# xbpeng/DeepTerrainRL

Hardware: AMD Instinct MI355X
Metric: env-steps/sec (batched rollout) dog/slopes_mixed (higher is better)
Workload: dtype f64

## Files before the change

### deepterrainrl_amd/csrc/dtrl_kernel_fast.h

```cpp
#pragma once
#include "dtrl_kernel.h"
#include "dtrl_topo.h"
#include <type_traits>

#if defined(__HIP_DEVICE_COMPILE__)

#if !DTRL_WAVE_SYNC
#error "dtrl_kernel_fast.h: the register-resident path is ONE wavefront per env by construction (v_readlane broadcasts, ballots, and LDS read-then-write sequences such as warm_match_fast() that rely on a wave's LDS operations completing in issue order). -DDTRL_WAVE_SYNC=0 builds the lane-phase reference path only (ADVICE r5)"
#endif

namespace dtrl {

__device__ __forceinline__ int lane_id() { return static_cast<int>(threadIdx.x); }
__device__ __forceinline__ int opaque_lane()
{
	int lane = static_cast<int>(threadIdx.x);
	asm volatile("" : "+v"(lane));
	return lane;
}
template <class T>
__device__ __forceinline__ void pin_loaded(T& v) { asm volatile("" : "+v"(v)); }
#if defined(DTRL_REAL_F32)
#define DTRL_VFMA "v_fma_f32"
#define DTRL_VMOV "v_mov_b32"
#else
#define DTRL_VFMA "v_fma_f64"
#define DTRL_VMOV "v_mov_b64"
#endif
__device__ __forceinline__ real bcast(real v, int src)
{
#if defined(DTRL_REAL_F32)
	return __int_as_float(__builtin_amdgcn_readlane(__float_as_int(v), src));
#else
	int lo = __builtin_amdgcn_readlane(__double2loint(v), src);
	int hi = __builtin_amdgcn_readlane(__double2hiint(v), src);
	return __hiloint2double(hi, lo);
#endif
}

template <int D>
__device__ __forceinline__ void mass_row(WSFast& ws, real (&h)[D])
{
	constexpr int Lk = D - 2;
	constexpr int kTab = Lk * (Lk + 5) / 2;
	constexpr int kFill = (kTab + 1) & ~1;
	static_assert(kFill <= static_cast<int>(sizeof(ws.Apk) / sizeof(real)), "mass table does not fit the packed-matrix storage");
	const int d = static_cast<int>(threadIdx.x);
	const int l = d >= 2 ? d - 2 : 0;
	const bool hinge = d >= 2 && d < D;
	real* T = ws.Apk;
	{
		struct alignas(2 * sizeof(real)) real2 { real x, y; };
		real2* T2 = reinterpret_cast<real2*>(T);
		const real2 z2 = {0.0, 0.0};
#pragma unroll
		for (int e = 0; e < (kFill / 2 + kGroup - 1) / kGroup; ++e) if (d + e * kGroup < kFill / 2) T2[d + e * kGroup] = z2;
	}
	env_sync();
	if (hinge) {
		const int base = l * (l + 5) / 2;
		const real m = ws.sm[l], mx = ws.smx[l], my = ws.smy[l];
		T[base] = -(my - m * ws.py[l]);
		T[base + 1] = (mx - m * ws.px[l]);
	}
	const int n_pairs = ws.M.n_pairs;
#pragma unroll 2
	for (int e = lane_id(); e < n_pairs; e += kGroup) {
		const int pl = ws.M.pair_l[e], pk = ws.M.pair_k[e];
		const int a = ws.M.path[pl][pk];
		const real m = ws.sm[pl], mx = ws.smx[pl], my = ws.smy[pl], I = ws.sI[pl];
		const real plx = ws.px[pl], ply = ws.py[pl];
		const real pax = ws.px[a], pay = ws.py[a];
		T[pl * (pl + 5) / 2 + 2 + a] = I - ((plx + pax) * mx + (ply + pay) * my) + m * (plx * pax + ply * pay);
	}
	env_sync();
	const real M0 = ws.sm[0];
	const real* Tl = T + (d < D ? d : 0);
	h[0] = (d == 0) ? M0 : 0.0;
	h[1] = (d == 1) ? M0 : 0.0;
#pragma unroll
	for (int c = 2; c < D; ++c) h[c] = Tl[(c - 2) * (c + 3) / 2];
	env_sync();
}

template <int B, int E, class F>
__device__ __forceinline__ void static_for(F&& f)
{
	if constexpr (B < E) { f(std::integral_constant<int, B>{}); static_for<B + 1, E>(f); }
}
template <int B, int E, class F>
__device__ __forceinline__ void static_for_down(F&& f)
{
	if constexpr (B < E) { f(std::integral_constant<int, E - 1>{}); static_for_down<B, E - 1>(f); }
}
template <int J>
__device__ __forceinline__ void fnma_lanes_ge(real& acc, real a, real b)
{
	unsigned long long sv, m;
	asm("s_lshl_b64 %2, -1, %5\n\ts_and_saveexec_b64 %1, %2\n\t" DTRL_VFMA " %0, -%3, %4, %0\n\ts_mov_b64 exec, %1"
	    : "+v"(acc), "=&s"(sv), "=&s"(m) : "v"(a), "s"(b), "n"(J) : "scc");
}
template <int I>
__device__ __forceinline__ void fnma_lanes_lt(real& acc, real a, real b)
{
	unsigned long long sv, m;
	asm("s_bfm_b64 %2, %5, 0\n\ts_and_saveexec_b64 %1, %2\n\t" DTRL_VFMA " %0, -%3, %4, %0\n\ts_mov_b64 exec, %1"
	    : "+v"(acc), "=&s"(sv), "=&s"(m) : "v"(a), "s"(b), "n"(I) : "scc");
}
template <int K>
__device__ __forceinline__ void mov_lane_eq(real& dst, real src)
{
	unsigned long long sv, m;
	asm("s_lshl_b64 %2, 1, %4\n\ts_and_saveexec_b64 %1, %2\n\t" DTRL_VMOV " %0, %3\n\ts_mov_b64 exec, %1"
	    : "+v"(dst), "=&s"(sv), "=&s"(m) : "v"(src), "n"(K) : "scc");
}
template <int I>
__device__ __forceinline__ void mov_lanes_lt(real& dst, real src)
{
	unsigned long long sv, m;
	asm("s_bfm_b64 %2, %4, 0\n\ts_and_saveexec_b64 %1, %2\n\t" DTRL_VMOV " %0, %3\n\ts_mov_b64 exec, %1"
	    : "+v"(dst), "=&s"(sv), "=&s"(m) : "v"(src), "n"(I) : "scc");
}
template <int B, int E>
__device__ __forceinline__ void mov_lanes_in(real& dst, real src)
{
	static_assert(0 <= B && B < E && E <= 64 && E - B < 64, "lane window (s_bfm_b64 takes the width modulo 64)");
	unsigned long long sv, m;
	asm("s_bfm_b64 %2, %4, %5\n\ts_and_saveexec_b64 %1, %2\n\t" DTRL_VMOV " %0, %3\n\ts_mov_b64 exec, %1"
	    : "+v"(dst), "=&s"(sv), "=&s"(m) : "v"(src), "n"(E - B), "n"(B) : "scc");
}
__device__ __forceinline__ void lds_store_ordered(real& dst, real v)
{
	dst = v;
	asm volatile("" : : : "memory");
}

template <class Topo>
__device__ __forceinline__ real factorize_regs(WSFast& ws, real (&h)[Topo::L + 2])
{
	constexpr int D = Topo::L + 2;
	const int lane = static_cast<int>(threadIdx.x);
	real dinv = 0;
	static_for_down<1, D>([&](auto kc) {
		constexpr int k = decltype(kc)::value;
		const real dk = bcast(h[k], k);
		const real ak = h[k];
		const real rk = fast_recip(dk);
		mov_lane_eq<k>(dinv, rk);
		const real lik = ak * rk;
		static_for_down<0, k>([&](auto jc) {
			constexpr int j = decltype(jc)::value;
			if constexpr (dof_coupled<Topo>(j, k)) h[j] = fmadd(-lik, bcast(ak, j), h[j]);
		});
		mov_lanes_lt<k>(h[k], lik);
	});
	{ const real r0 = fast_recip(h[0]); if (lane == 0) dinv = r0; }
	static_assert((D - 1) * (D - 2) / 2 + kGroup - 1 < static_cast<int>(sizeof(ws.Apk) / sizeof(real)), "the unpredicated store of U's last column leaves the packed-matrix storage");
	real* S = ws.Apk;
	static_for<1, D>([&](auto kc) {
		constexpr int k = decltype(kc)::value;
		lds_store_ordered(S[k * (k - 1) / 2 + lane], h[k]);
	});
	env_sync();
	const int base = lane < D ? lane * (lane - 1) / 2 : 0;
	static_for<0, D - 1>([&](auto kc) {
		constexpr int k = decltype(kc)::value;
		const real t = S[base + k];
		mov_lanes_in<k + 1, D>(h[k], t);
	});
	env_sync();
	return dinv;
}
template <int D>
__device__ __forceinline__ real usolve_regs(const real (&h)[D], real z)
{
	static_for_down<1, D>([&](auto kc) {
		constexpr int k = decltype(kc)::value;
		const real zk = bcast(z, k);
		fnma_lanes_lt<k>(z, h[k], zk);
	});
	return z;
}
template <class Topo>
constexpr int first_update_col(int i)
{
	for (int k = Topo::L + 1; k > i; --k) if (dof_coupled<Topo>(i, k)) return k;
	return 0;
}
template <class Topo, int kAhead = 1>
__device__ __forceinline__ void usolve_rows(WSFast& ws, int R)
{
	constexpr int D = Topo::L + 2;
	const int lane = static_cast<int>(threadIdx.x);
	if (lane > R) return;
	real* z = ws.Z[lane];
	const real* U = ws.Apk;
	real acc[D], u[D * (D - 1) / 2];
	auto fetch = [&](auto kc) {
		constexpr int k = decltype(kc)::value;
		static_for<0, k>([&](auto ic) {
			constexpr int i = decltype(ic)::value;
			if constexpr (dof_coupled<Topo>(i, k)) u[k * (k - 1) / 2 + i] = U[k * (k - 1) / 2 + i];
			if constexpr (first_update_col<Topo>(i) == k) acc[i] = z[i];
		});
		if constexpr (first_update_col<Topo>(k) == 0) acc[k] = z[k];
	};
	static_for_down<D - kAhead, D>(fetch);
	static_for_down<1, D>([&](auto kc) {
		constexpr int k = decltype(kc)::value;
		__builtin_amdgcn_sched_barrier(0);
		if constexpr (k - kAhead >= 1) fetch(std::integral_constant<int, k - kAhead>{});
		const real zk = acc[k];
		if constexpr (first_update_col<Topo>(k) != 0) z[k] = zk;
		static_for_down<0, k>([&](auto ic) {
			constexpr int i = decltype(ic)::value;
			if constexpr (dof_coupled<Topo>(i, k)) acc[i] = fmadd(-u[k * (k - 1) / 2 + i], zk, acc[i]);
		});
	});
	z[0] = acc[0];
}
template <int D>
__device__ __forceinline__ real utsolve_regs(const real (&h)[D], real u)
{
	static_for<0, D - 1>([&](auto kc) {
		constexpr int k = decltype(kc)::value;
		const real uk = bcast(u, k);
		fnma_lanes_ge<k + 1>(u, h[k], uk);
	});
	return u;
}

static_assert((kMaxPts + kGroup - 1) / kGroup == 3, "written for up to 3 sample points per lane");
constexpr int pts_per_lane(int L) { return (L * kPtsPerLink + kGroup - 1) / kGroup; }
struct ContactPts { PtVal p0, p1, p2; unsigned long long m0, m1, m2;  unsigned long long f0, f1, f2;  };
template <int NP>
__device__ __forceinline__ unsigned link_field(unsigned long long m0, unsigned long long m1, unsigned long long m2, int link)
{
	const int b = link * kPtsPerLink, word = b >> 6, off = b & 63;
	unsigned long long lo = m0, hi = NP > 1 ? m1 : 0ull;
	if constexpr (NP > 1) if (word == 1) { lo = m1; hi = NP > 2 ? m2 : 0ull; }
	if constexpr (NP > 2) if (word == 2) { lo = m2; hi = 0ull; }
	unsigned long long bits = lo >> off;
	if (off + kPtsPerLink > 64) bits |= hi << (64 - off);
	return static_cast<unsigned>(bits & ((1ull << kPtsPerLink) - 1ull));
}
constexpr real kNoPoint = -1.0e30;
template <int NP>
__device__ __noinline__ unsigned link_cap_drop_mask(WSFast& ws, real d0, real d1, real d2)
{
	const int lane = opaque_lane();
	const int npts = ws.M.L * kPtsPerLink;
	real* S = ws.Apk;
	if (lane < npts) S[lane] = d0;
	if constexpr (NP > 1) if (lane + kGroup < npts) S[lane + kGroup] = d1;
	if constexpr (NP > 2) if (lane + 2 * kGroup < npts) S[lane + 2 * kGroup] = d2;
	env_sync();
	auto over = [&](real d, int pt) -> unsigned {
		if (!(d > kNoPoint)) return 0u;
		const int base = (pt / kPtsPerLink) * kPtsPerLink;
		int rank = 0;
		for (int k = 0; k < kPtsPerLink; ++k) { const int o = base + k; const real od = S[o]; rank += (o != pt && (od > d || (od == d && o < pt))) ? 1 : 0; }
		return rank >= kMaxPtsPerLink ? 1u : 0u;
	};
	unsigned m = over(d0, lane);
	if constexpr (NP > 1) m |= over(d1, lane + kGroup) << 1;
	if constexpr (NP > 2) m |= over(d2, lane + 2 * kGroup) << 2;
	env_sync();
	return m;
}
template <int L, bool kFlags>
__device__ __forceinline__ ContactPts eval_points(WSFast& ws, const DevModel& gm, const GroundRec& g)
{
	constexpr int NP = pts_per_lane(L), npts = L * kPtsPerLink;
	const int lane = opaque_lane();
	const GroundHdr gh = ground_header(g);
	const real q0 = ws.st.q[0], q1 = ws.st.q[1];
	const real tol = kFlags ? gm.contact_tol : real(0);
	bool have[NP]; int col[NP]; real lx[NP], ly[NP], margin[NP], brk[NP], cs[NP], sn[NP], px[NP], py[NP];
	static_for<0, NP>([&](auto ec) {
		constexpr int e = decltype(ec)::value;
		const int pt = lane + e * kGroup;
		have[e] = (e + 1) * kGroup <= npts || pt < npts;
		const int ptc = ((e + 1) * kGroup <= npts || pt < npts) ? pt : npts - 1;
		const int j = ptc / kPtsPerLink;
		col[e] = ws.M.col[j];
		cs[e] = ws.cs[j]; sn[e] = ws.sn[j]; px[e] = ws.px[j]; py[e] = ws.py[j];
		const real* lp = &gm.pt_ground[0][0][0] + 2 * ptc;
		lx[e] = lp[0]; ly[e] = lp[1];
		margin[e] = gm.link_margin[j]; brk[e] = gm.link_brk[j];
	});
	static_for<0, NP>([&](auto ec) {
		constexpr int e = decltype(ec)::value;
		pin_loaded(col[e]); pin_loaded(lx[e]); pin_loaded(ly[e]); pin_loaded(margin[e]); pin_loaded(brk[e]);
	});
	real x[NP], y[NP]; GroundCell cell[NP];
	static_for<0, NP>([&](auto ec) {
		constexpr int e = decltype(ec)::value;
		x[e] = px[e] + cs[e] * lx[e] - sn[e] * ly[e];
		y[e] = py[e] + sn[e] * lx[e] + cs[e] * ly[e];
		cell[e] = ground_cell(gh, q0 + x[e]);
	});
	real ha[NP], hb[NP];
	static_for<0, NP>([&](auto ec) {
		constexpr int e = decltype(ec)::value;
		ha[e] = g.data[cell[e].seg][cell[e].i];
		hb[e] = g.data[cell[e].seg][cell[e].j];
	});
	PtVal r[3];
	static_for<0, 3>([&](auto ec) {
		constexpr int e = decltype(ec)::value;
		r[e].x = 0; r[e].y = 0; r[e].depth = 0; r[e].nx = 0; r[e].ny = 0; r[e].active = 0; r[e].near = 0;
		if constexpr (e < NP) {
			real slope;
			const real h = ground_height(cell[e], ha[e], hb[e], &slope);
			const real gap = h - (q1 + y[e]);
			const bool in_reach = kFlags || (gap + (margin[e] + brk[e]) * (1.0 + fabs(slope)) > 0);
			const real inv = fast_rsqrt(1.0 + slope * slope);
			const real depth = fmadd(gap, inv, margin[e]);
			const bool live = have[e] & (col[e] != 0);
			if (kFlags) r[e].near = (live & (depth >= -tol)) ? 1 : 0;
			r[e].active = (live & in_reach & (depth > -brk[e])) ? 1 : 0;
			r[e].nx = -slope * inv; r[e].ny = inv;
			r[e].depth = depth;
			r[e].x = x[e]; r[e].y = y[e];
		}
	});
	ContactPts c;
	c.p0 = r[0]; c.p1 = r[1]; c.p2 = r[2];
	c.f0 = 0; c.f1 = 0; c.f2 = 0;
	if (kFlags) { c.f0 = __ballot(c.p0.near); if constexpr (NP > 1) c.f1 = __ballot(c.p1.near); if constexpr (NP > 2) c.f2 = __ballot(c.p2.near); }
	c.m0 = __ballot(c.p0.active); c.m1 = 0; c.m2 = 0;
	if constexpr (NP > 1) c.m1 = __ballot(c.p1.active);
	if constexpr (NP > 2) c.m2 = __ballot(c.p2.active);
	if ((c.m0 | c.m1 | c.m2) != 0ull) {
		const int many = (lane < L) && __popc(link_field<NP>(c.m0, c.m1, c.m2, lane)) > kMaxPtsPerLink;
		if (__builtin_expect(__ballot(many) != 0ull, 0)) {
			const unsigned drop = link_cap_drop_mask<NP>(ws, c.p0.active ? c.p0.depth : kNoPoint, (NP > 1 && c.p1.active) ? c.p1.depth : kNoPoint, (NP > 2 && c.p2.active) ? c.p2.depth : kNoPoint);
			if (drop & 1u) c.p0.active = 0;
			if (drop & 2u) c.p1.active = 0;
			if (drop & 4u) c.p2.active = 0;
			c.m0 = __ballot(c.p0.active);
			if constexpr (NP > 1) c.m1 = __ballot(c.p1.active);
			if constexpr (NP > 2) c.m2 = __ballot(c.p2.active);
		}
	}
	return c;
}
template <int NP>
__device__ __noinline__ unsigned row_cap_drop_mask(WSFast& ws, real d0, real d1, real d2, int cap)
{
	const int lane = opaque_lane();
	const int npts = ws.M.L * kPtsPerLink;
	real* S = ws.Apk;
	if (lane < npts) S[lane] = d0;
	if constexpr (NP > 1) if (lane + kGroup < npts) S[lane + kGroup] = d1;
	if constexpr (NP > 2) if (lane + 2 * kGroup < npts) S[lane + 2 * kGroup] = d2;
	env_sync();
	auto over = [&](real d, int pt) -> unsigned {
		if (!(d > kNoPoint)) return 0u;
		int rank = 0;
		for (int o = 0; o < npts; ++o) { const real od = S[o]; rank += (o != pt && (od > d || (od == d && o < pt))) ? 1 : 0; }
		return rank >= cap ? 1u : 0u;
	};
	unsigned m = over(d0, lane);
	if constexpr (NP > 1) m |= over(d1, lane + kGroup) << 1;
	if constexpr (NP > 2) m |= over(d2, lane + 2 * kGroup) << 2;
	env_sync();
	return m;
}
__device__ __forceinline__ unsigned long long pairs_in_reach(const WSFast& ws)
{
	const int lane = static_cast<int>(threadIdx.x);
	return __ballot(lane < ws.M.n_cpairs && pair_in_reach(ws, lane));
}
constexpr int kPairCands = 2 * kPtsPerLink, kPairSlots = kGroup / kPairCands;
__device__ __noinline__ int append_pair_rows_fast(WSFast& ws, const DevModel& gm, int R, unsigned long long reach)
{
	const int lane = opaque_lane();
	const unsigned long long below = (lane == 0) ? 0ull : (~0ull >> (64 - lane));
	const int slot = lane / kPairCands, cand = lane - slot * kPairCands;
	while (reach != 0ull && R + 2 <= kMaxRows) {
		int mypr = -1;
#pragma unroll
		for (int sidx = 0; sidx < kPairSlots; ++sidx) {
			if (reach != 0ull) { const int pr = __ffsll(static_cast<long long>(reach)) - 1; reach &= reach - 1ull; if (slot == sidx) mypr = pr; }
		}
		int P = 0, Q = 0, k = 0;
		PairHit hit; hit.active = 0; hit.depth = 0; hit.x = 0; hit.y = 0; hit.nx = 0; hit.ny = 0;
		if (mypr >= 0) { pair_candidate(ws.M.cp_a[mypr], ws.M.cp_b[mypr], cand, &P, &Q, &k); hit = pair_point_eval(ws, gm, P, Q, k); }
		const unsigned long long am = __ballot(hit.active);
		if (am == 0ull) continue;
		int keep = hit.active;
		const int mine_cnt = __popcll((am >> (slot * kPairCands)) & ((1ull << kPairCands) - 1ull));
		if (__builtin_expect(__ballot(lane < kPairSlots * kPairCands && mine_cnt > kMaxPtsPerPair) != 0ull, 0)) {
			real* S = ws.Apk;
			S[lane] = hit.active ? hit.depth : -1.0;
			env_sync();
			if (hit.active) {
				int rank = 0;
				for (int o = 0; o < kPairCands; ++o) { const real od = S[slot * kPairCands + o]; rank += (o != cand && od > 0 && (od > hit.depth || (od == hit.depth && o < cand))) ? 1 : 0; }
				keep = rank < kMaxPtsPerPair;
			}
			env_sync();
		}
		const unsigned long long km = __ballot(keep);
		const int room = (kMaxRows - R) / 2;
		const int idx = __popcll(km & below);
		if (keep && idx < room) {
			const int Rw = R + 2 * idx;
			ws.row_kind[Rw] = 1; ws.row_link[Rw] = P; ws.row_link2[Rw] = static_cast<int8_t>(Q); ws.row_x[Rw] = hit.x; ws.row_y[Rw] = hit.y;
			ws.row_dx[Rw] = hit.nx; ws.row_dy[Rw] = hit.ny; ws.row_tgt[Rw] = 0;
			ws.row_id[Rw] = pair_row_id(mypr, cand, 0); ws.row_id[Rw + 1] = pair_row_id(mypr, cand, 1);
			ws.row_kind[Rw + 1] = 2; ws.row_link[Rw + 1] = P; ws.row_link2[Rw + 1] = static_cast<int8_t>(Q); ws.row_x[Rw + 1] = hit.x; ws.row_y[Rw + 1] = hit.y;
			ws.row_dx[Rw + 1] = hit.ny; ws.row_dy[Rw + 1] = -hit.nx; ws.row_tgt[Rw + 1] = 0;
		}
		int n = __popcll(km); if (n > room) n = room;
		R += 2 * n;
	}
	return R;
}
template <int NP>
__device__ __forceinline__ void contact_bits_fast(WSFast& ws, unsigned long long m0, unsigned long long m1, unsigned long long m2)
{
	const int lane = static_cast<int>(threadIdx.x);
	int any = 0;
	if (lane < ws.M.L) any = link_field<NP>(m0, m1, m2, lane) != 0u;
	const unsigned long long lm = __ballot(any);
	if (lane == 0) ws.st.contact_bits = static_cast<uint32_t>(lm);
}
__device__ __forceinline__ void emit_contact_rows(WSFast& ws, const PtVal& p, int pt, int rank, int cap, int R0, real inv_h)
{
	if (p.active && rank < cap) {
		const int R = R0 + 2 * rank;
		const int j = pt / kPtsPerLink;
		ws.row_kind[R] = 1; ws.row_link[R] = j; ws.row_link2[R] = -1; ws.row_x[R] = p.x; ws.row_y[R] = p.y;
		ws.row_dx[R] = p.nx; ws.row_dy[R] = p.ny; ws.row_tgt[R] = normal_row_target(p.depth, inv_h);
		ws.row_id[R] = ground_row_id(pt, 0); ws.row_id[R + 1] = ground_row_id(pt, 1);
		ws.row_kind[R + 1] = 2; ws.row_link[R + 1] = j; ws.row_link2[R + 1] = -1; ws.row_x[R + 1] = p.x; ws.row_y[R + 1] = p.y;
		ws.row_dx[R + 1] = p.ny; ws.row_dy[R + 1] = -p.nx; ws.row_tgt[R + 1] = 0;
	}
}
template <int NP>
__device__ __forceinline__ void build_rows_fast(WSFast& ws, const DevModel& gm, const ContactPts& c_in, real h)
{
	ContactPts c = c_in;
	const int lane = opaque_lane();
	const unsigned long long below = (lane == 0) ? 0ull : (~0ull >> (64 - lane));
	const real inv_h = 1.0 / h;
	int lim = 0; real tgt = 0;
	if (lane >= 1 && lane < ws.M.L && !(ws.M.lim_lo[lane] > ws.M.lim_hi[lane])) {
		const real th = ws.st.q[lane + 2];
		if (th <= ws.M.lim_lo[lane] + kLimitSlop) { lim = 1; tgt = kLimitErp * fmax(ws.M.lim_lo[lane] - th, 0.0) * inv_h; }
		else if (th >= ws.M.lim_hi[lane] - kLimitSlop) { lim = -1; tgt = kLimitErp * fmax(th - ws.M.lim_hi[lane], 0.0) * inv_h; }
	}
	const unsigned long long ml = __ballot(lim != 0);
	const int rl = __popcll(ml & below);
	int R0 = __popcll(ml); if (R0 > kMaxRows) R0 = kMaxRows;
	if (lim != 0 && rl < kMaxRows) { ws.row_kind[rl] = 0; ws.row_link[rl] = lane; ws.row_link2[rl] = -1; ws.row_dx[rl] = lim; ws.row_tgt[rl] = tgt; ws.row_id[rl] = kNoRowId; }
	const int cap = (kMaxRows - R0) / 2;
	if (__builtin_expect(__popcll(c.m0) + __popcll(c.m1) + __popcll(c.m2) > cap, 0)) {
		const unsigned drop = row_cap_drop_mask<NP>(ws, c.p0.active ? c.p0.depth : kNoPoint, (NP > 1 && c.p1.active) ? c.p1.depth : kNoPoint, (NP > 2 && c.p2.active) ? c.p2.depth : kNoPoint, cap);
		if (drop & 1u) c.p0.active = 0;
		if (drop & 2u) c.p1.active = 0;
		if (drop & 4u) c.p2.active = 0;
		c.m0 = __ballot(c.p0.active);
		if constexpr (NP > 1) c.m1 = __ballot(c.p1.active);
		if constexpr (NP > 2) c.m2 = __ballot(c.p2.active);
	}
	const int n0 = __popcll(c.m0), n1 = __popcll(c.m1), n2 = __popcll(c.m2);
	emit_contact_rows(ws, c.p0, lane, __popcll(c.m0 & below), cap, R0, inv_h);
	if constexpr (NP > 1) emit_contact_rows(ws, c.p1, lane + kGroup, n0 + __popcll(c.m1 & below), cap, R0, inv_h);
	if constexpr (NP > 2) emit_contact_rows(ws, c.p2, lane + 2 * kGroup, n0 + n1 + __popcll(c.m2 & below), cap, R0, inv_h);
	int nc = n0 + n1 + n2; if (nc > cap) nc = cap;
	int R = R0 + 2 * nc;
	const unsigned long long reach = pairs_in_reach(ws);
	if (__builtin_expect(reach != 0ull, 0)) R = append_pair_rows_fast(ws, gm, R, reach);
	if (lane == 0) ws.R = R;
	env_sync();
}

template <int D>
__device__ __forceinline__ void build_delassus_fast(WSFast& ws, real h, real dinv_mine)
{
	const int lane = static_cast<int>(threadIdx.x);
	const int R = ws.R;
	const int n_ent = R * (R + 1) / 2;
	if (R < 16) {
		typedef v4r_t v4d_t;
		const int g = lane >> 4, c = lane & 15;
		real jv = 0;
		if (lane < R) {
			const int sw = lane;
			if (ws.row_kind[sw] == 0) jv = ws.row_dx[sw] * ws.st.qd[ws.row_link[sw] + 2];
			else jv = row_point_jv(ws, sw);
		}
		const int zrow = c <= R ? c : 0;
		v4d_t acc = {0, 0, 0, 0};
#pragma unroll
		for (int s4 = 0; s4 < (D + 3) / 4; ++s4) {
			const int k = 4 * s4 + g;
			const bool live = k < D;
			const real z = ws.Z[zrow][live ? k : 0], dk = ws.dinv[live ? k : 0];
			const real b = live ? z : 0.0;
			const real a = live ? z * dk : 0.0;
			acc = mfma_16x16x4(a, b, acc);
		}
#pragma unroll
		for (int r = 0; r < 4; ++r) {
			const int i = mfma_row(r, g);
			if (i < R && c <= i) ws.Apk[i * (i + 1) / 2 + c] = acc[r];
			if (i < R && c == R) ws.wv[i] = acc[r];
		}
		env_sync();
		if (lane < R) ws.wv[lane] = jv + h * ws.wv[lane] - ws.row_tgt[lane];
		env_sync();
		return;
	}
	const real* di = ws.dinv;
	auto entry_rows = [](int e, int& s, int& r) {
		s = static_cast<int>((sqrtf(8.0f * e + 1.0f) - 1.0f) * 0.5f);
		while (s * (s + 1) / 2 > e) --s;
		while ((s + 1) * (s + 2) / 2 <= e) ++s;
		r = e - s * (s + 1) / 2;
	};
	{
		const bool has_e = lane < n_ent, has_w = lane < R;
		int s = 0, r = 0;
		if (has_e) entry_rows(lane, s, r);
		const int sw = has_w ? lane : 0;
		real jv = 0;
		if (has_w) {
			if (ws.row_kind[sw] == 0) jv = ws.row_dx[sw] * ws.st.qd[ws.row_link[sw] + 2];
			else jv = row_point_jv(ws, sw);
		}
		const real* zs = ws.Z[s];
		const real* zr = ws.Z[r];
		const real* zw = ws.Z[sw];
		const real* z0 = ws.Z[R];
		real a = 0, zz = 0;
#pragma unroll 4
		for (int i = 0; i < D; ++i) { a = fmadd(zs[i] * di[i], zr[i], a); zz = fmadd(zw[i] * di[i], z0[i], zz); }
		if (has_e) ws.Apk[lane] = a;
		if (has_w) ws.wv[lane] = jv + h * zz - ws.row_tgt[lane];
	}
	for (int e = lane + kGroup; e < n_ent; e += kGroup) {
		int s, r; entry_rows(e, s, r);
		const real* zs = ws.Z[s];
		const real* zr = ws.Z[r];
		real a = 0;
#pragma unroll 4
		for (int i = 0; i < D; ++i) a = fmadd(zs[i] * di[i], zr[i], a);
		ws.Apk[e] = a;
	}
	env_sync();
}

__device__ __forceinline__ real wave_shr1(real v)
{
#if defined(DTRL_REAL_F32)
	return __int_as_float(__builtin_amdgcn_update_dpp(0, __float_as_int(v), 0x138, 0xf, 0xf, false));
#else
	const int lo = __builtin_amdgcn_update_dpp(0, __double2loint(v), 0x138, 0xf, 0xf, false);
	const int hi = __builtin_amdgcn_update_dpp(0, __double2hiint(v), 0x138, 0xf, 0xf, false);
	return __hiloint2double(hi, lo);
#endif
}
enum PgsRowKind { kPgsRowNormal, kPgsRowFriction, kPgsRowGeneric };
template <PgsRowKind kKind>
__device__ __forceinline__ void pgs_row_step(real& w, real& lam, real rinv, real a_sr, int r, int lane, bool tang, real lo, real hi)
{
	real nl;
	if constexpr (kKind == kPgsRowGeneric) {
		const real lim = kMu * wave_shr1(lam);
		const real glo = tang ? -lim : 0.0, ghi = tang ? lim : __builtin_huge_val();
		nl = fmin(fmax(fmadd(-w, rinv, lam), glo), ghi);
	} else {
		nl = fmadd(-w, rinv, lam);
		if constexpr (kKind == kPgsRowFriction) nl = fmin(fmax(nl, lo), hi); else nl = fmax(nl, 0.0);
	}
	const real dl = bcast(nl - lam, r);
	if (lane == r) lam = nl;
	w = fmadd(a_sr, dl, w);
}
template <int r, int K>
__device__ __forceinline__ void pgs_rows_load(real (&a)[K], const WSFast& ws, int lane, bool mine, int R)
{
	if constexpr (r < K) {
		if (r < R) {
			const int mx = lane > r ? lane : r, mn = lane < r ? lane : r;
			a[r] = ws.Apk[mine ? mx * (mx + 1) / 2 + mn : 0];
			pgs_rows_load<r + 1, K>(a, ws, lane, mine, R);
		}
	}
}
template <int r, int K>
__device__ __forceinline__ void pgs_rows_sweep(const real (&a)[K], real& w, real& lam, real rinv, bool tang, unsigned long long actR, int lane, int R)
{
	if constexpr (r < K) {
		if (r < R) {
			if ((actR >> r) & 1ull) pgs_row_step<kPgsRowGeneric>(w, lam, rinv, a[r], r, lane, tang, 0.0, 0.0);
			pgs_rows_sweep<r + 1, K>(a, w, lam, rinv, tang, actR, lane, R);
		}
	}
}
template <PgsRowKind kKind, int r, int K>
__device__ __forceinline__ void pgs_rows_pass(const real (&a)[K], real& w, real& lam, real rinv, real lo, real hi, unsigned long long rows, int lane, int R)
{
	if constexpr (r < K) {
		if (r < R) {
			if ((rows >> r) & 1ull) pgs_row_step<kKind>(w, lam, rinv, a[r], r, lane, false, lo, hi);
			pgs_rows_pass<kKind, r + 1, K>(a, w, lam, rinv, lo, hi, rows, lane, R);
		}
	}
}
template <int r, int K>
__device__ __forceinline__ void pgs_rows_warm(const real (&a)[K], real& w, real lam, unsigned long long nz, int R)
{
	if constexpr (r < K) {
		if (r < R) {
			if ((nz >> r) & 1ull) w = fmadd(a[r], bcast(lam, r), w);
			pgs_rows_warm<r + 1, K>(a, w, lam, nz, R);
		}
	}
}
__device__ __forceinline__ void warm_match_fast(WSFast& ws)
{
	const int lane = opaque_lane();
	const int R = ws.R, Rp = ws.st.ws_R;
	if (R == 0) { if (Rp != 0 && lane == 0) ws.st.ws_R = 0; return; }
	int id = kNoRowId;
	if (lane < R) id = ws.row_id[lane];
	real l0 = 0.0;
	if (ws.M.warm_start != 0 && Rp > 0) {
		int hit = -1;
		for (int p = 0; p < Rp; ++p) hit = (ws.st.ws_id[p] == id) ? p : hit;
		if (id < kFirstPairRowId && hit >= 0) l0 = kWarmFactor * ws.st.ws_lam[hit];
	}
	if (lane < R) { ws.st.ws_lam[lane] = l0; ws.st.ws_id[lane] = static_cast<uint16_t>(id); }
	if (lane == 0) ws.st.ws_R = R;
}
template <int kPgsRegRows>
__device__ __forceinline__ void pgs_solve_fast(WSFast& ws)
{
	const int lane = opaque_lane();
	const int R = ws.R;
	const bool mine = lane < R;
	real w = mine ? ws.wv[lane] : 0.0;
	real rinv = 0.0;
	if (mine) { const real ass = ws.Apk[lane * (lane + 3) / 2]; rinv = (ass >= 1e-12) ? 1.0 / ass : 0.0; }
	real lam = (mine && rinv != 0.0) ? ws.st.ws_lam[lane] : 0.0;
	const bool tang = mine && ws.row_kind[lane] == 2;
	const unsigned long long act = __ballot(rinv != 0.0);
	const bool warm = ws.M.warm_start != 0;
	const unsigned long long tmask = __ballot(tang);
	const unsigned long long nz_l0 = __ballot(lam != 0.0);
	const bool any_l0 = nz_l0 != 0ull;
	if (kPgsRegRows == kMaxRows || R <= kPgsRegRows) {
		real a[kPgsRegRows];
		pgs_rows_load<0, kPgsRegRows>(a, ws, lane, mine, R);
		const unsigned long long actR = act & ((R < 64) ? ((1ull << R) - 1ull) : ~0ull);
		if (any_l0) pgs_rows_warm<0, kPgsRegRows>(a, w, lam, nz_l0, R);
		const unsigned long long pass0 = warm ? (actR & ~tmask) : actR, pass1 = actR & tmask;
		if (warm) {
			const int end0 = (pass0 == 0ull) ? R : 64 - __builtin_clzll(pass0);
#pragma unroll 1
			for (int it = 0; it < kPgsIters; ++it) {
				unsigned rows0_lo = static_cast<unsigned>(pass0), rows0_hi = static_cast<unsigned>(pass0 >> 32); int last0 = end0;
				asm volatile("" : "+s"(rows0_lo), "+s"(rows0_hi), "+s"(last0));
				const unsigned long long rows0 = (static_cast<unsigned long long>(rows0_hi) << 32) | rows0_lo;
				if (rows0 != 0ull) pgs_rows_pass<kPgsRowNormal, 0, kPgsRegRows>(a, w, lam, rinv, 0.0, 0.0, rows0, lane, last0);
				const real ln = wave_shr1(lam);
				const real lim = kMu * ln;
				const unsigned long long rows = pass1 & __ballot(tang && ln > kHoldEps);
				if (rows != 0ull) pgs_rows_pass<kPgsRowFriction, 0, kPgsRegRows>(a, w, lam, rinv, -lim, lim, rows, lane, 64 - __builtin_clzll(rows));
			}
		} else {
#pragma unroll 1
			for (int it = 0; it < kPgsIters; ++it) {
				unsigned rows_lo = static_cast<unsigned>(actR), rows_hi = static_cast<unsigned>(actR >> 32); int last = R;
#if defined(DTRL_REAL_F32)
				asm volatile("" : "+s"(rows_lo), "+s"(rows_hi));
#else
				asm volatile("" : "+s"(rows_lo), "+s"(rows_hi), "+s"(last));
#endif
				pgs_rows_sweep<0, kPgsRegRows>(a, w, lam, rinv, tang, (static_cast<unsigned long long>(rows_hi) << 32) | rows_lo, lane, last);
			}
		}
		if (mine) ws.st.ws_lam[lane] = lam;
		env_sync();
		return;
	}
	const int tri = lane * (lane + 1) / 2;
	if (any_l0) for (int r = 0; r < R; ++r) if ((nz_l0 >> r) & 1ull) { const int mx = lane > r ? lane : r, mn = lane < r ? lane : r; w = fmadd(ws.Apk[mine ? mx * (mx + 1) / 2 + mn : 0], bcast(lam, r), w); }
	real a_nx = mine ? ws.Apk[tri] : 0.0;
	const unsigned long long actR = act & ((R < 64) ? ((1ull << R) - 1ull) : ~0ull);
	if (warm) {
		const unsigned long long pass0 = actR & ~tmask, pass1 = actR & tmask;
		for (int it = 0; it < kPgsIters; ++it) {
			for (int r = 0; r < R; ++r) {
				const real a_sr = a_nx;
				const int rn = (r + 1 < R) ? r + 1 : 0;
				{ const int mx = lane > rn ? lane : rn, mn = lane < rn ? lane : rn; a_nx = ws.Apk[mine ? mx * (mx + 1) / 2 + mn : 0]; }
				if (!((pass0 >> r) & 1ull)) continue;
				pgs_row_step<kPgsRowNormal>(w, lam, rinv, a_sr, r, lane, false, 0.0, 0.0);
			}
			const real ln = wave_shr1(lam);
			const real lim = kMu * ln;
			const unsigned long long rows = pass1 & __ballot(tang && ln > kHoldEps);
			for (int r = 0; r < R; ++r) {
				const real a_sr = a_nx;
				const int rn = (r + 1 < R) ? r + 1 : 0;
				{ const int mx = lane > rn ? lane : rn, mn = lane < rn ? lane : rn; a_nx = ws.Apk[mine ? mx * (mx + 1) / 2 + mn : 0]; }
				if (!((rows >> r) & 1ull)) continue;
				pgs_row_step<kPgsRowFriction>(w, lam, rinv, a_sr, r, lane, false, -lim, lim);
			}
		}
	} else {
		for (int it = 0; it < kPgsIters; ++it) {
			for (int r = 0; r < R; ++r) {
				const real a_sr = a_nx;
				const int rn = (r + 1 < R) ? r + 1 : 0;
				{ const int mx = lane > rn ? lane : rn, mn = lane < rn ? lane : rn; a_nx = ws.Apk[mine ? mx * (mx + 1) / 2 + mn : 0]; }
				if (!((act >> r) & 1ull)) continue;
				pgs_row_step<kPgsRowGeneric>(w, lam, rinv, a_sr, r, lane, tang, 0.0, 0.0);
			}
		}
	}
	if (mine) ws.st.ws_lam[lane] = lam;
	env_sync();
}

constexpr int kKinBatch = 3;
template <class Topo>
__device__ __forceinline__ void kin_dyn_terms_fast(WSFast& ws)
{
	constexpr int L = Topo::L, kDepth = topo_depth<Topo>();
	static_assert(kDepth >= 2 && kDepth <= kMaxDepth, "path length of the skeleton against the model's path table");
	constexpr int kWords = (kDepth + 3) / 4;
	PROF_T0();
	const int lane = opaque_lane();
	const bool mine = lane < L;
	const int j = mine ? lane : 0;
	const int dep = ws.M.depth[j], pa = ws.M.parent[j];
	uint32_t pw[kWords];
#pragma unroll
	for (int t = 0; t < kWords; ++t) pw[t] = path_word(ws, j, t);
	const int mc = lane & 15;
	const uint32_t m0_l = ws.M.sub_mask[mc < L ? mc : 0], m1_l = ws.M.sub_mask[16 + mc < L ? 16 + mc : 0];
	const real at0 = ws.M.attach[j][0], at1 = ws.M.attach[j][1], ba0 = ws.M.body_attach[j][0], ba1 = ws.M.body_attach[j][1];
	const real m = ws.M.mass[j], inr = ws.M.inertia[j], subm = ws.M.sub_mass[j];
	int a[kDepth];
#pragma unroll
	for (int k = 0; k < kDepth; ++k) a[k] = (k <= dep) ? static_cast<int>((pw[k / 4] >> (8 * (k % 4))) & 0xffu) : 0;
	real qa[kDepth], wa[kDepth];
#pragma unroll
	for (int k = 0; k < kDepth; ++k) { qa[k] = ws.st.q[a[k] + 2]; wa[k] = ws.st.qd[a[k] + 2]; }
	const real vx0 = ws.st.qd[0], vy0 = ws.st.qd[1];
#pragma unroll
	for (int k = 0; k < kDepth; ++k) { pin_loaded(qa[k]); pin_loaded(wa[k]); }
	real phi = 0, w = 0;
#pragma unroll
	for (int k = 0; k < kDepth; ++k) {
		const real on = (k <= dep) ? 1.0 : 0.0;
		phi = fmadd(qa[k], on, phi); w = fmadd(wa[k], on, w);
	}
	real sn, cs; sincos_r(phi, &sn, &cs);
	if (mine) { ws.phi[j] = phi; ws.w[j] = w; ws.cs[j] = cs; ws.sn[j] = sn; }
	env_sync();
	PROF_ADD(ws, kProfP1);
	{
		const int pc = pa >= 0 ? pa : 0;
		const real c = ws.cs[pc], s = ws.sn[pc], wp = ws.w[pc];
		const real rx = c * at0 - s * at1;
		const real ry = s * at0 + c * at1;
		const real ux = -(wp * ry), uy = wp * rx;
		const real w2 = wp * wp;
		const real gx = -(w2 * rx), gy = -(w2 * ry);
		const bool has = pa >= 0;
		if (mine) {
			ws.bx[j] = has ? rx : 0.0; ws.by[j] = has ? ry : 0.0; ws.ux[j] = has ? ux : 0.0; ws.uy[j] = has ? uy : 0.0; ws.gx[j] = has ? gx : 0.0; ws.gy[j] = has ? gy : 0.0;
		}
	}
	env_sync();
	PROF_ADD(ws, kProfP2);
	real px = 0, py = 0, vx = vx0, vy = vy0, ax = 0, ay = 0;
	{
		constexpr int kN = kDepth - 1;
		real v[kN][6];
		auto load = [&](int k) {
			const int e = a[k];
			v[k - 1][0] = ws.bx[e]; v[k - 1][1] = ws.by[e]; v[k - 1][2] = ws.ux[e]; v[k - 1][3] = ws.uy[e]; v[k - 1][4] = ws.gx[e]; v[k - 1][5] = ws.gy[e];
		};
#pragma unroll
		for (int k = 1; k <= (kKinBatch < kN ? kKinBatch : kN); ++k) load(k);
		__builtin_amdgcn_sched_barrier(0);
#pragma unroll
		for (int b0 = 1; b0 <= kN; b0 += kKinBatch) {
#pragma unroll
			for (int k = b0 + kKinBatch; k < b0 + 2 * kKinBatch && k <= kN; ++k) load(k);
			__builtin_amdgcn_sched_barrier(0);
#pragma unroll
			for (int k = b0; k < b0 + kKinBatch && k <= kN; ++k) {
#pragma unroll
				for (int t = 0; t < 6; ++t) pin_loaded(v[k - 1][t]);
			}
#pragma unroll
			for (int k = b0; k < b0 + kKinBatch && k <= kN; ++k) {
				const real on = (k <= dep) ? 1.0 : 0.0;
				px = fmadd(v[k - 1][0], on, px); py = fmadd(v[k - 1][1], on, py); vx = fmadd(v[k - 1][2], on, vx); vy = fmadd(v[k - 1][3], on, vy);
				ax = fmadd(v[k - 1][4], on, ax); ay = fmadd(v[k - 1][5], on, ay);
			}
		}
		if constexpr (kDepth < kMaxDepth) { vx = vx + 0.0; vy = vy + 0.0; }
	}
	{
		const real ax0 = 0, ay0 = -kGravityY;
		const real rx = cs * ba0 - sn * ba1;
		const real ry = sn * ba0 + cs * ba1;
		const real cx = px + rx, cy = py + ry;
		const real w2 = w * w;
		const real fx = m * ((ax0 + ax) - w2 * rx), fy = m * ((ay0 + ay) - w2 * ry);
		if (mine) {
			ws.px[j] = px; ws.py[j] = py; ws.vpx[j] = vx; ws.vpy[j] = vy;
			ws.cx[j] = cx; ws.cy[j] = cy;
			ws.vcx[j] = vx - w * ry; ws.vcy[j] = vy + w * rx;
			ws.fx[j] = fx; ws.fy[j] = fy; ws.fn[j] = cx * fy - cy * fx;
			ws.mcx[j] = m * cx; ws.mcy[j] = m * cy; ws.Io[j] = inr + m * (cx * cx + cy * cy);
		}
	}
	env_sync();
	PROF_ADD(ws, kProfP3);
	{
		const int g = lane >> 4, c = lane & 15;
		const real* V = &ws.fx[0];
		const uint32_t m0 = (c < L) ? m0_l : 0u, m1 = (16 + c < L) ? m1_l : 0u;
		real bv[kMaxL / 4];
#pragma unroll
		for (int s4 = 0; s4 < kMaxL / 4; ++s4) {
			const int k = 4 * s4 + g;
			const bool live = (c < 6) & (k < L);
			bv[s4] = V[live ? c * kMaxL + k : 0];
		}
#pragma unroll
		for (int s4 = 0; s4 < kMaxL / 4; ++s4) pin_loaded(bv[s4]);
		v4r_t acc0 = {0, 0, 0, 0}, acc1 = {0, 0, 0, 0};
#pragma unroll
		for (int s4 = 0; s4 < kMaxL / 4; ++s4) {
			const int k = 4 * s4 + g;
			const bool live = (c < 6) & (k < L);
			const real b = live ? bv[s4] : 0.0;
			const real a0 = ((m0 >> k) & 1u) ? 1.0 : 0.0, a1 = ((m1 >> k) & 1u) ? 1.0 : 0.0;
			acc0 = mfma_16x16x4(a0, b, acc0);
			acc1 = mfma_16x16x4(a1, b, acc1);
		}
		if (c < 6) {
			real* out = (c < 3) ? &ws.sfs[c][0] : (&ws.smx[0] + (c - 3) * kMaxL);
#pragma unroll
			for (int r = 0; r < 4; ++r) {
				const int j0 = mfma_row(r, g), j1 = 16 + mfma_row(r, g);
				if (j0 < L) out[j0] = acc0[r];
				if (j1 < L) out[j1] = acc1[r];
			}
		}
	}
	env_sync();
	{
		const real sfx = ws.sfs[0][j], sfy = ws.sfs[1][j], sfn = ws.sfs[2][j];
		const real bl = sfn - px * sfy + py * sfx;
		if (mine) {
			ws.sm[j] = subm;
			ws.b[j + 2] = bl;
			if (j == 0) { ws.b[0] = sfx; ws.b[1] = sfy; }
		}
	}
	env_sync();
	PROF_ADD(ws, kProfP4);
}

#if defined(DTRL_PROFILE)
__device__ __forceinline__ int prof_row_bucket(int R) { return R == 0 ? 0 : (R <= 6 ? 1 : (R <= 12 ? 2 : (R <= 18 ? 3 : 4))); }
#endif
template <class Topo>
struct FastPath {
	static constexpr int D = Topo::L + 2;
	static constexpr int NP = pts_per_lane(Topo::L);
	static __device__ void substep(WSFast& ws, const DevModel& gm, const GroundRec& g, real h, bool kin_valid)
	{
		const int lane = static_cast<int>(threadIdx.x);
#if defined(DTRL_PROFILE)
		const unsigned long long prof_sub_t0 = __builtin_readcyclecounter();
#endif
		if (!kin_valid) { PROF_T0(); kin_dyn_terms_fast<Topo>(ws); PROF_ADD(ws, kProfFK); }
		const int rows_ready = kin_valid ? ws.n_pts_active : -1;
		if (rows_ready >= 0) {
			if (lane == 0) { ws.R = rows_ready; ws.n_pts_active = -1; }
			env_sync();
		} else {
			ContactPts cp;
			{ PROF_T0(); cp = eval_points<Topo::L, false>(ws, gm, g); PROF_ADD(ws, kProfDetect); }
			{ PROF_T0(); build_rows_fast<NP>(ws, gm, cp, h); PROF_ADD(ws, kProfRows); }
		}
		{ PROF_T0(); warm_match_fast(ws); PROF_ADD(ws, kProfRows); }
		real hrow[D];
		{ PROF_T0(); mass_row<D>(ws, hrow); PROF_ADD(ws, kProfMass); }
		real dinv;
		{ PROF_T0(); dinv = factorize_regs<Topo>(ws, hrow); PROF_ADD(ws, kProfFact); }
		const int R = ws.R;
		if (lane == 0) ws.cost += 8 + R;
		{
			PROF_T0();
			const bool hinge = lane >= 2 && lane < D;
			const real mypx = hinge ? ws.px[lane - 2] : 0.0, mypy = hinge ? ws.py[lane - 2] : 0.0;
			const uint32_t mysub = hinge ? ws.M.sub_mask[lane - 2] : 0u;
			real rhs0 = (lane < D) ? (ws.st.tau[lane] - ws.b[lane]) : 0.0;
			if (__builtin_expect(ws.st.pert_on != 0, 0)) { if (lane < D) rhs0 += perturb_gen_force(ws, lane); }
			if (R < 1) {
				if (0 <= R) {
					const real z = usolve_regs<D>(hrow, rhs0);
					if (lane < D) ws.Z[0][lane] = z;
				}
			} else {
				{
					const int ol = opaque_lane();
					const int rc = ol < R ? ol : 0;
					const int kind_l = ws.row_kind[rc], link_l = ws.row_link[rc], link2_l = ws.row_link2[rc];
					const real dx_l = ws.row_dx[rc], dy_l = ws.row_dy[rc], x_l = ws.row_x[rc], y_l = ws.row_y[rc];
					for (int r = 0; r < R; ++r) {
						const int kind = __builtin_amdgcn_readlane(kind_l, r), link = __builtin_amdgcn_readlane(link_l, r);
						const real dx = bcast(dx_l, r);
						real v;
						if (kind == 0) v = (lane == link + 2) ? dx : 0.0;
						else {
							const real dy = bcast(dy_l, r), x = bcast(x_l, r), y = bcast(y_l, r);
							const int link2 = __builtin_amdgcn_readlane(link2_l, r);
							const int on = static_cast<int>((mysub >> link) & 1u) - (link2 < 0 ? 0 : static_cast<int>((mysub >> link2) & 1u));
							const real jr = dx * (-(y - mypy)) + dy * (x - mypx);
							v = on == 0 ? 0.0 : (on > 0 ? jr : -jr);
							v = (lane == 0) ? (link2 < 0 ? dx : 0.0) : v;
							v = (lane == 1) ? (link2 < 0 ? dy : 0.0) : v;
						}
						if (lane < D) ws.Z[r][lane] = v;
					}
					if (lane < D) ws.Z[R][lane] = rhs0;
				}
				env_sync();
				usolve_rows<Topo>(ws, R);
			}
			if (lane < D) ws.dinv[lane] = dinv;
			env_sync();
			PROF_ADD(ws, kProfFsub);
#if defined(DTRL_PROFILE)
			PROF_ADD(ws, kProfFsubR0 + prof_row_bucket(R));
#endif
		}
		if (R > 0) {
			{ PROF_T0(); build_delassus_fast<D>(ws, h, dinv); PROF_ADD(ws, kProfDelassus); }
			{ PROF_T0(); pgs_solve_fast<Topo::kPgsRegRows>(ws); PROF_ADD(ws, kProfPgs); }
		}
		{
			PROF_T0();
			real u = 0;
			if (lane < D) {
				real s = h * ws.Z[R][lane];
				for (int r = 0; r < R; ++r) s = fmadd(ws.Z[r][lane], ws.st.ws_lam[r], s);
				u = s * dinv;
			}
			u = utsolve_regs<D>(hrow, u);
			if (lane < D) { const real v = clamp_turn_rate(ws.st.qd[lane] + u, lane, h); ws.st.qd[lane] = v; ws.st.q[lane] += h * v; }
			env_sync();
			PROF_ADD(ws, kProfFinish);
		}
#if defined(DTRL_PROFILE)
		if (threadIdx.x == 0) { ws.prof[kProfRowsSum] += R; ws.prof[kProfSubsteps] += 1; const int bk = prof_row_bucket(R); ws.prof[kProfR0 + bk] += 1; ws.prof[kProfT0 + bk] += __builtin_readcyclecounter() - prof_sub_t0; }
#endif
	}
	static __device__ void kinematics(WSFast& ws) { kin_dyn_terms_fast<Topo>(ws); }
	static __device__ void pd_solve(WSFast& ws, real dt)
	{
		const int lane = static_cast<int>(threadIdx.x);
		real hrow[D];
		mass_row<D>(ws, hrow);
		const real add = (lane < D) ? dt * ws.kdm[lane] : 0.0;
#pragma unroll
		for (int k = 0; k < D; ++k) if (lane == k) hrow[k] += add;
		const real dinv = factorize_regs<Topo>(ws, hrow);
		real z = (lane < D) ? ws.u[lane] : 0.0;
		z = usolve_regs<D>(hrow, z);
		real u = z * dinv;
		u = utsolve_regs<D>(hrow, u);
		env_sync();
		if (lane < D) ws.u[lane] = u;
		if (lane == 0) ws.R = 0;
		env_sync();
	}
	static __device__ void contacts(WSFast& ws, const DevModel& gm, const GroundRec& g, real h)
	{
		const ContactPts cp = eval_points<Topo::L, true>(ws, gm, g);
		contact_bits_fast<NP>(ws, cp.f0, cp.f1, cp.f2);
		build_rows_fast<NP>(ws, gm, cp, h);
		if (threadIdx.x == 0) ws.n_pts_active = ws.R;
		env_sync();
	}
};

}
#endif
```

Baseline: 21.27 million.

## Compact PGS rows into slot order, pass values in registers, batch LDS loads

Reorders the warm-start PGS solve so active normal and friction rows are packed into contiguous register slots, with a ds_permute slot map, instead of iterating over sparse row masks. This is gated by a per-topology WavesPerEu trait. The Delassus build now computes jv branch-free, batches its LDS loads before the MFMA chain, and returns w in a register so PGS does not re-read it. warm_match now runs after factorization using scalar R/Rp/warm values and readlane broadcasts instead of repeated LDS reads. The aim is to cut LDS latency and divergent row iteration, at the cost of more registers and added code complexity.

Result: faster. 21.75 million (median of 6 runs) (+2.2%).

```diff
diff --git a/deepterrainrl_amd/csrc/dtrl_kernel_fast.h b/deepterrainrl_amd/csrc/dtrl_kernel_fast.h
--- a/deepterrainrl_amd/csrc/dtrl_kernel_fast.h
+++ b/deepterrainrl_amd/csrc/dtrl_kernel_fast.h
@@ -20,6 +20,7 @@
 }
 template <class T>
 __device__ __forceinline__ void pin_loaded(T& v) { asm volatile("" : "+v"(v)); }
+__device__ __forceinline__ void lds_loads_arrived() { __builtin_amdgcn_s_waitcnt(0xc07f); }
 #if defined(DTRL_REAL_F32)
 #define DTRL_VFMA "v_fma_f32"
 #define DTRL_VMOV "v_mov_b32"
@@ -480,29 +481,44 @@
 }
 
 template <int D>
-__device__ __forceinline__ void build_delassus_fast(WSFast& ws, real h, real dinv_mine)
+__device__ __forceinline__ real build_delassus_fast(WSFast& ws, real h, real dinv_mine, int R)
 {
 	const int lane = static_cast<int>(threadIdx.x);
-	const int R = ws.R;
 	const int n_ent = R * (R + 1) / 2;
 	if (R < 16) {
 		typedef v4r_t v4d_t;
 		const int g = lane >> 4, c = lane & 15;
-		real jv = 0;
-		if (lane < R) {
-			const int sw = lane;
-			if (ws.row_kind[sw] == 0) jv = ws.row_dx[sw] * ws.st.qd[ws.row_link[sw] + 2];
-			else jv = row_point_jv(ws, sw);
+		real jv, tgt;
+		{
+			const int ol = opaque_lane();
+			const int rc = ol < R ? ol : 0;
+			const int kind_l = ws.row_kind[rc], link_l = ws.row_link[rc], link2_l = ws.row_link2[rc];
+			const real dx_l = ws.row_dx[rc], dy_l = ws.row_dy[rc], x_l = ws.row_x[rc], y_l = ws.row_y[rc];
+			tgt = ws.row_tgt[rc];
+			const int l2c = link2_l < 0 ? 0 : link2_l;
+			const real qd_l = ws.st.qd[link_l + 2];
+			const real jv1 = link_point_vel(ws, link_l, x_l, y_l, dx_l, dy_l), jv2 = link_point_vel(ws, l2c, x_l, y_l, dx_l, dy_l);
+			const real jp = link2_l < 0 ? jv1 : jv1 - jv2;
+			jv = kind_l == 0 ? dx_l * qd_l : jp;
 		}
 		const int zrow = c <= R ? c : 0;
-		v4d_t acc = {0, 0, 0, 0};
-#pragma unroll
-		for (int s4 = 0; s4 < (D + 3) / 4; ++s4) {
+		constexpr int kSteps = (D + 3) / 4;
+		real zv[kSteps], dv[kSteps];
+#pragma unroll
+		for (int s4 = 0; s4 < kSteps; ++s4) {
 			const int k = 4 * s4 + g;
 			const bool live = k < D;
-			const real z = ws.Z[zrow][live ? k : 0], dk = ws.dinv[live ? k : 0];
-			const real b = live ? z : 0.0;
-			const real a = live ? z * dk : 0.0;
+			zv[s4] = ws.Z[zrow][live ? k : 0]; dv[s4] = ws.dinv[live ? k : 0];
+		}
+#pragma unroll
+		for (int s4 = 0; s4 < kSteps; ++s4) { pin_loaded(zv[s4]); pin_loaded(dv[s4]); }
+		v4d_t acc = {0, 0, 0, 0};
+#pragma unroll
+		for (int s4 = 0; s4 < kSteps; ++s4) {
+			const int k = 4 * s4 + g;
+			const bool live = k < D;
+			const real b = live ? zv[s4] : 0.0;
+			const real a = live ? zv[s4] * dv[s4] : 0.0;
 			acc = mfma_16x16x4(a, b, acc);
 		}
 #pragma unroll
@@ -512,9 +528,10 @@
 			if (i < R && c == R) ws.wv[i] = acc[r];
 		}
 		env_sync();
-		if (lane < R) ws.wv[lane] = jv + h * ws.wv[lane] - ws.row_tgt[lane];
+		real w = 0.0;
+		if (lane < R) { w = jv + h * ws.wv[lane] - tgt; ws.wv[lane] = w; }
 		env_sync();
-		return;
+		return w;
 	}
 	const real* di = ws.dinv;
 	auto entry_rows = [](int e, int& s, int& r) {
@@ -523,6 +540,7 @@
 		while ((s + 1) * (s + 2) / 2 <= e) ++s;
 		r = e - s * (s + 1) / 2;
 	};
+	real w = 0.0;
 	{
 		const bool has_e = lane < n_ent, has_w = lane < R;
 		int s = 0, r = 0;
@@ -541,7 +559,7 @@
 #pragma unroll 4
 		for (int i = 0; i < D; ++i) { a = fmadd(zs[i] * di[i], zr[i], a); zz = fmadd(zw[i] * di[i], z0[i], zz); }
 		if (has_e) ws.Apk[lane] = a;
-		if (has_w) ws.wv[lane] = jv + h * zz - ws.row_tgt[lane];
+		if (has_w) { w = jv + h * zz - ws.row_tgt[lane]; ws.wv[lane] = w; }
 	}
 	for (int e = lane + kGroup; e < n_ent; e += kGroup) {
 		int s, r; entry_rows(e, s, r);
@@ -553,6 +571,7 @@
 		ws.Apk[e] = a;
 	}
 	env_sync();
+	return w;
 }
 
 __device__ __forceinline__ real wave_shr1(real v)
@@ -623,56 +642,128 @@
 		}
 	}
 }
-__device__ __forceinline__ void warm_match_fast(WSFast& ws)
+__device__ __forceinline__ real pgs_slot_entry(const WSFast& ws, int lane, bool mine, int row)
+{
+	const int mx = lane > row ? lane : row, mn = lane < row ? lane : row;
+	return ws.Apk[mine ? mx * (mx + 1) / 2 + mn : 0];
+}
+template <int j, int K>
+__device__ __forceinline__ void pgs_slots_load_up(real (&a)[K], const WSFast& ws, int lane, bool mine, int srow, int n0)
+{
+	if constexpr (j < K) {
+		if (j < n0) {
+			a[j] = pgs_slot_entry(ws, lane, mine, __builtin_amdgcn_readlane(srow, j));
+			pgs_slots_load_up<j + 1, K>(a, ws, lane, mine, srow, n0);
+		}
+	}
+}
+template <int j, int K>
+__device__ __forceinline__ void pgs_slots_load_down(real (&a)[K], const WSFast& ws, int lane, bool mine, int srow, int n1)
+{
+	if constexpr (j < K) {
+		if (j < n1) {
+			a[K - 1 - j] = pgs_slot_entry(ws, lane, mine, __builtin_amdgcn_readlane(srow, K - 1 - j));
+			pgs_slots_load_down<j + 1, K>(a, ws, lane, mine, srow, n1);
+		}
+	}
+}
+template <int j, int K>
+__device__ __forceinline__ void pgs_slots_pass0(const real (&a)[K], real& w, real& lam, real rinv, int lane, int srow, int n0)
+{
+	if constexpr (j < K) {
+		if (j < n0) {
+			pgs_row_step<kPgsRowNormal>(w, lam, rinv, a[j], __builtin_amdgcn_readlane(srow, j), lane, false, 0.0, 0.0);
+			pgs_slots_pass0<j + 1, K>(a, w, lam, rinv, lane, srow, n0);
+		}
+	}
+}
+template <int j, int K>
+__device__ __forceinline__ void pgs_slots_pass1(const real (&a)[K], real& w, real& lam, real rinv, real lo, real hi, int lane, int srow, int n1, unsigned long long rows)
+{
+	if constexpr (j < K) {
+		if (j < n1) {
+			const int row = __builtin_amdgcn_readlane(srow, K - 1 - j);
+			if ((rows >> row) & 1ull) pgs_row_step<kPgsRowFriction>(w, lam, rinv, a[K - 1 - j], row, lane, false, lo, hi);
+			pgs_slots_pass1<j + 1, K>(a, w, lam, rinv, lo, hi, lane, srow, n1, rows);
+		}
+	}
+}
+__device__ __forceinline__ void warm_match_fast(WSFast& ws, int R, int Rp, bool warm)
 {
 	const int lane = opaque_lane();
-	const int R = ws.R, Rp = ws.st.ws_R;
 	if (R == 0) { if (Rp != 0 && lane == 0) ws.st.ws_R = 0; return; }
-	int id = kNoRowId;
-	if (lane < R) id = ws.row_id[lane];
+	const int own = ws.row_id[lane < R ? lane : 0];
+	const int cached = ws.st.ws_id[lane < Rp ? lane : 0];
+	const int id = lane < R ? own : kNoRowId;
 	real l0 = 0.0;
-	if (ws.M.warm_start != 0 && Rp > 0) {
+	if (warm && Rp > 0) {
 		int hit = -1;
-		for (int p = 0; p < Rp; ++p) hit = (ws.st.ws_id[p] == id) ? p : hit;
-		if (id < kFirstPairRowId && hit >= 0) l0 = kWarmFactor * ws.st.ws_lam[hit];
+		for (int p = 0; p < Rp; ++p) hit = (__builtin_amdgcn_readlane(cached, p) == id) ? p : hit;
+		const real lh = ws.st.ws_lam[hit >= 0 ? hit : 0];
+		if (id < kFirstPairRowId && hit >= 0) l0 = kWarmFactor * lh;
 	}
 	if (lane < R) { ws.st.ws_lam[lane] = l0; ws.st.ws_id[lane] = static_cast<uint16_t>(id); }
 	if (lane == 0) ws.st.ws_R = R;
 }
-template <int kPgsRegRows>
-__device__ __forceinline__ void pgs_solve_fast(WSFast& ws)
+template <int kPgsRegRows, bool kSlotOrder>
+__device__ __forceinline__ void pgs_solve_fast(WSFast& ws, int R, bool warm, real w)
 {
 	const int lane = opaque_lane();
-	const int R = ws.R;
 	const bool mine = lane < R;
-	real w = mine ? ws.wv[lane] : 0.0;
+	const int rc = mine ? lane : 0;
+	const real ass = ws.Apk[rc * (rc + 3) / 2], lam_ws = ws.st.ws_lam[rc];
+	const int kind = ws.row_kind[rc];
 	real rinv = 0.0;
-	if (mine) { const real ass = ws.Apk[lane * (lane + 3) / 2]; rinv = (ass >= 1e-12) ? 1.0 / ass : 0.0; }
-	real lam = (mine && rinv != 0.0) ? ws.st.ws_lam[lane] : 0.0;
-	const bool tang = mine && ws.row_kind[lane] == 2;
+	if (mine) rinv = (ass >= 1e-12) ? 1.0 / ass : 0.0;
+	real lam = (mine && rinv != 0.0) ? lam_ws : 0.0;
+	const bool tang = mine && kind == 2;
 	const unsigned long long act = __ballot(rinv != 0.0);
-	const bool warm = ws.M.warm_start != 0;
 	const unsigned long long tmask = __ballot(tang);
 	const unsigned long long nz_l0 = __ballot(lam != 0.0);
 	const bool any_l0 = nz_l0 != 0ull;
 	if (kPgsRegRows == kMaxRows || R <= kPgsRegRows) {
 		real a[kPgsRegRows];
-		pgs_rows_load<0, kPgsRegRows>(a, ws, lane, mine, R);
+		if (!kSlotOrder || !warm || any_l0) pgs_rows_load<0, kPgsRegRows>(a, ws, lane, mine, R);
+		lds_loads_arrived();
 		const unsigned long long actR = act & ((R < 64) ? ((1ull << R) - 1ull) : ~0ull);
 		if (any_l0) pgs_rows_warm<0, kPgsRegRows>(a, w, lam, nz_l0, R);
 		const unsigned long long pass0 = warm ? (actR & ~tmask) : actR, pass1 = actR & tmask;
 		if (warm) {
-			const int end0 = (pass0 == 0ull) ? R : 64 - __builtin_clzll(pass0);
+			if constexpr (kSlotOrder) {
+				const int n0 = __popcll(pass0), n1 = __popcll(pass1);
+				int srow;
+				{
+					const unsigned long long below = (1ull << lane) - 1ull;
+					const bool has = ((actR >> lane) & 1ull) != 0ull;
+					const int slot = tang ? kPgsRegRows - 1 - __popcll(pass1 & below) : __popcll(pass0 & below);
+					srow = __builtin_amdgcn_ds_permute((has ? slot : 63) << 2, lane);
+				}
+				pgs_slots_load_up<0, kPgsRegRows>(a, ws, lane, mine, srow, n0);
+				pgs_slots_load_down<0, kPgsRegRows>(a, ws, lane, mine, srow, n1);
+				lds_loads_arrived();
 #pragma unroll 1
-			for (int it = 0; it < kPgsIters; ++it) {
-				unsigned rows0_lo = static_cast<unsigned>(pass0), rows0_hi = static_cast<unsigned>(pass0 >> 32); int last0 = end0;
-				asm volatile("" : "+s"(rows0_lo), "+s"(rows0_hi), "+s"(last0));
-				const unsigned long long rows0 = (static_cast<unsigned long long>(rows0_hi) << 32) | rows0_lo;
-				if (rows0 != 0ull) pgs_rows_pass<kPgsRowNormal, 0, kPgsRegRows>(a, w, lam, rinv, 0.0, 0.0, rows0, lane, last0);
-				const real ln = wave_shr1(lam);
-				const real lim = kMu * ln;
-				const unsigned long long rows = pass1 & __ballot(tang && ln > kHoldEps);
-				if (rows != 0ull) pgs_rows_pass<kPgsRowFriction, 0, kPgsRegRows>(a, w, lam, rinv, -lim, lim, rows, lane, 64 - __builtin_clzll(rows));
+				for (int it = 0; it < kPgsIters; ++it) {
+					int n0s = n0, n1s = n1, srows = srow;
+					asm volatile("" : "+s"(n0s), "+s"(n1s), "+v"(srows));
+					pgs_slots_pass0<0, kPgsRegRows>(a, w, lam, rinv, lane, srows, n0s);
+					const real ln = wave_shr1(lam);
+					const real lim = kMu * ln;
+					const unsigned long long rows = pass1 & __ballot(tang && ln > kHoldEps);
+					if (rows != 0ull) pgs_slots_pass1<0, kPgsRegRows>(a, w, lam, rinv, -lim, lim, lane, srows, n1s, rows);
+				}
+			} else {
+				const int end0 = (pass0 == 0ull) ? R : 64 - __builtin_clzll(pass0);
+#pragma unroll 1
+				for (int it = 0; it < kPgsIters; ++it) {
+					unsigned rows0_lo = static_cast<unsigned>(pass0), rows0_hi = static_cast<unsigned>(pass0 >> 32); int last0 = end0;
+					asm volatile("" : "+s"(rows0_lo), "+s"(rows0_hi), "+s"(last0));
+					const unsigned long long rows0 = (static_cast<unsigned long long>(rows0_hi) << 32) | rows0_lo;
+					if (rows0 != 0ull) pgs_rows_pass<kPgsRowNormal, 0, kPgsRegRows>(a, w, lam, rinv, 0.0, 0.0, rows0, lane, last0);
+					const real ln = wave_shr1(lam);
+					const real lim = kMu * ln;
+					const unsigned long long rows = pass1 & __ballot(tang && ln > kHoldEps);
+					if (rows != 0ull) pgs_rows_pass<kPgsRowFriction, 0, kPgsRegRows>(a, w, lam, rinv, -lim, lim, rows, lane, 64 - __builtin_clzll(rows));
+				}
 			}
 		} else {
 #pragma unroll 1
@@ -880,6 +971,8 @@
 #if defined(DTRL_PROFILE)
 __device__ __forceinline__ int prof_row_bucket(int R) { return R == 0 ? 0 : (R <= 6 ? 1 : (R <= 12 ? 2 : (R <= 18 ? 3 : 4))); }
 #endif
+template <class Topo> struct WavesPerEu;
+template <class Topo> struct PgsSlotOrder { static constexpr bool value = WavesPerEu<Topo>::value <= 2; };
 template <class Topo>
 struct FastPath {
 	static constexpr int D = Topo::L + 2;
@@ -900,12 +993,13 @@
 			{ PROF_T0(); cp = eval_points<Topo::L, false>(ws, gm, g); PROF_ADD(ws, kProfDetect); }
 			{ PROF_T0(); build_rows_fast<NP>(ws, gm, cp, h); PROF_ADD(ws, kProfRows); }
 		}
-		{ PROF_T0(); warm_match_fast(ws); PROF_ADD(ws, kProfRows); }
 		real hrow[D];
 		{ PROF_T0(); mass_row<D>(ws, hrow); PROF_ADD(ws, kProfMass); }
 		real dinv;
 		{ PROF_T0(); dinv = factorize_regs<Topo>(ws, hrow); PROF_ADD(ws, kProfFact); }
-		const int R = ws.R;
+		const int R = __builtin_amdgcn_readfirstlane(ws.R), Rp = __builtin_amdgcn_readfirstlane(ws.st.ws_R);
+		const bool warm = __builtin_amdgcn_readfirstlane(ws.M.warm_start) != 0;
+		{ PROF_T0(); warm_match_fast(ws, R, Rp, warm); PROF_ADD(ws, kProfRows); }
 		if (lane == 0) ws.cost += 8 + R;
 		{
 			PROF_T0();
@@ -954,8 +1048,9 @@
 #endif
 		}
 		if (R > 0) {
-			{ PROF_T0(); build_delassus_fast<D>(ws, h, dinv); PROF_ADD(ws, kProfDelassus); }
-			{ PROF_T0(); pgs_solve_fast<Topo::kPgsRegRows>(ws); PROF_ADD(ws, kProfPgs); }
+			real w;
+			{ PROF_T0(); w = build_delassus_fast<D>(ws, h, dinv, R); PROF_ADD(ws, kProfDelassus); }
+			{ PROF_T0(); pgs_solve_fast<Topo::kPgsRegRows, PgsSlotOrder<Topo>::value>(ws, R, warm, w); PROF_ADD(ws, kProfPgs); }
 		}
 		{
 			PROF_T0();
```
